# microsoft/DCVC

Measured on AMD Instinct MI355X. Metric: 1080p YUV420 intra encode+decode pictures per second (DCVC-UF-Intra (DMCI), real rANS bit streams, q_index in {0,16,32,48,63}; sequential loop: compress then decompress per picture), higher is better.
Workload: dtype f16

## Files before the change

dcvc_amd/csrc/codec/codec_base.h:

```cpp
#pragma once

#include "codec/modules.h"
#include "rans/rans_coder.h"

#include <initializer_list>
#include <condition_variable>
#include <functional>
#include <map>
#include <mutex>
#include <thread>

namespace dcvc {

constexpr int kMinSymbolsPerStream = 32768;
constexpr int kQpNum = 64;

inline int ceil_div(int a, int b) { return (a + b - 1) / b; }
inline int ec_parallel_for(int symbols)
{
    const int p = symbols / kMinSymbolsPerStream;
    return p < 1 ? 1 : (p > kMaxEcParallel ? kMaxEcParallel : p);
}

struct Geometry {
    int H8 = 0, W8 = 0, H16 = 0, W16 = 0, H16p = 0, W16p = 0, H32 = 0, W32 = 0, H64 = 0, W64 = 0;
    int P8() const { return H8 * W8; }
    int P16() const { return H16 * W16; }
    int P16p() const { return H16p * W16p; }
    int P32() const { return H32 * W32; }
    int P64() const { return H64 * W64; }
    bool padded() const { return H16p != H16 || W16p != W16; }

    static Geometry of(int height, int width)
    {
        Geometry g;
        g.H8 = ceil_div(height, 16) * 2; g.W8 = ceil_div(width, 16) * 2;
        g.H16 = g.H8 / 2; g.W16 = g.W8 / 2;
        g.H16p = ceil_div(g.H16, 4) * 4; g.W16p = ceil_div(g.W16, 4) * 4;
        g.H32 = g.H16p / 2; g.W32 = g.W16p / 2;
        g.H64 = g.H16p / 4; g.W64 = g.W16p / 4;
        return g;
    }
};

template <typename T>
class Pinned {
public:
    Pinned() = default;
    ~Pinned() { release(); }
    Pinned(const Pinned&) = delete;
    Pinned& operator=(const Pinned&) = delete;
    void reserve(size_t count)
    {
        if (count <= m_cap) return;
        release();
        hip_check(hipHostMalloc(reinterpret_cast<void**>(&m_p), count * sizeof(T), hipHostMallocDefault),
                  "hipHostMalloc");
        m_cap = count;
    }
    T* get() const { return m_p; }
    T& operator[](size_t i) const { return m_p[i]; }

private:
    void release()
    {
        if (m_p) (void)hipHostFree(m_p);
        m_p = nullptr;
        m_cap = 0;
    }
    T* m_p = nullptr;
    size_t m_cap = 0;
};

class CodecBase {
public:
    void set_use_graphs(bool on) { m_use_graphs = on; }
    const std::vector<uint8_t>& stream_bytes() const { return m_enc.stream(); }

protected:
    CodecBase();
    ~CodecBase();
    CodecBase(const CodecBase&) = delete;
    CodecBase& operator=(const CodecBase&) = delete;

    hipStream_t enter(hipStream_t user);
    void leave(hipStream_t user);

    template <typename F>
    void run_stage(int key, hipStream_t st, F&& fn);
    void bind_stage_arg(int key, const void* arg);
    void clear_graphs();
    void quiesce();

    void submit(hipStream_t st, std::function<void()> job);
    void wait_job();

    void load_cdf_tables(const ParamStore& ps);
    const half_t* upload_qp_table(const ParamStore& ps, DeviceArena& mem, const char* name, int ch);
    struct QpRow {
        half_t* dst;
        const half_t* table;
        int ch;
    };
    static void copy_qp_rows(std::initializer_list<QpRow> rows, int qp, hipStream_t st);

    void upload_code_length_tables(const ParamStore& ps, DeviceArena& mem, int ch_z, int max_n);
    void probe_code_length(int n, const int16_t* comp, long long comp_stride, int count, const int32_t* totals, int n_totals,
                           const int8_t* z, int nz, int qp, int64_t* units, int64_t* kept, hipStream_t st);

    RansEncoder m_enc;
    RansDecoder m_dec;
    hipStream_t m_io_stream = nullptr;
    hipStream_t m_cs = nullptr;
    hipStream_t m_join = nullptr;
    bool m_use_graphs = true;

private:
    const uint32_t *m_cl_y = nullptr, *m_cl_z = nullptr;
    int m_cl_y_num = 0, m_cl_z_num = 0, m_cl_ch_z = 0, m_cl_max_n = 0;
    unsigned long long* m_cl_sums = nullptr;
    Pinned<unsigned long long> m_h_cl;

    void worker_loop();

    struct GraphSlot {
        hipGraphExec_t exec = nullptr;
        bool warmed = false;
        const void* arg = nullptr;
    };
    std::map<int, GraphSlot> m_graphs;
    hipEvent_t m_ev_job = nullptr, m_ev_in = nullptr, m_ev_out = nullptr;
    std::thread m_worker;
    std::mutex m_mu;
    std::condition_variable m_cv_work, m_cv_done;
    std::function<void()> m_job;
    bool m_pending = false, m_done = true, m_stop = false;
    std::string m_worker_error;
};

template <typename F>
void CodecBase::run_stage(int key, hipStream_t st, F&& fn)
{
    if (!m_use_graphs) {
        fn();
        return;
    }
    GraphSlot& slot = m_graphs[key];
    if (!slot.warmed) {
        fn();
        slot.warmed = true;
        return;
    }
    if (!slot.exec) {
        hipGraph_t graph = nullptr;
// ... 18 lines not shown
```

dcvc_amd/csrc/codec/codec_base.hip:

```cpp
#include "codec/codec_base.h"

#include "rans/code_length.h"

#include <chrono>
#include <cstdio>
#include <cstdlib>
#include <string>

namespace dcvc {

CodecBase::CodecBase()
{
    int lo = 0, hi = 0;
    hip_check(hipDeviceGetStreamPriorityRange(&lo, &hi), "hipDeviceGetStreamPriorityRange");
    int prio = 0, io_prio = hi;
    if (const char* e = getenv("DCVC_COMPUTE_PRIORITY")) {
        const std::string v(e);
        prio = v == "high" ? hi : v == "low" ? lo : 0;
        io_prio = v == "low" ? lo : hi;
    }
    hip_check(hipStreamCreateWithPriority(&m_io_stream, hipStreamNonBlocking, io_prio), "hipStreamCreate(io)");
    hip_check(hipStreamCreateWithPriority(&m_cs, hipStreamNonBlocking, prio), "hipStreamCreate(compute)");
    hip_check(hipEventCreateWithFlags(&m_ev_job, hipEventDisableTiming), "hipEventCreate");
    hip_check(hipEventCreateWithFlags(&m_ev_in, hipEventDisableTiming), "hipEventCreate");
    hip_check(hipEventCreateWithFlags(&m_ev_out, hipEventDisableTiming), "hipEventCreate");
    m_worker = std::thread(&CodecBase::worker_loop, this);
}

CodecBase::~CodecBase()
{
    {
        std::lock_guard<std::mutex> lk(m_mu);
        m_stop = true;
    }
    m_cv_work.notify_all();
    if (m_worker.joinable()) m_worker.join();
    clear_graphs();
    if (m_cs) (void)hipStreamSynchronize(m_cs);
    if (m_ev_job) (void)hipEventDestroy(m_ev_job);
    if (m_ev_in) (void)hipEventDestroy(m_ev_in);
    if (m_ev_out) (void)hipEventDestroy(m_ev_out);
    if (m_join) (void)hipStreamDestroy(m_join);
    if (m_cs) (void)hipStreamDestroy(m_cs);
    if (m_io_stream) (void)hipStreamDestroy(m_io_stream);
}

void CodecBase::clear_graphs()
{
    for (auto& kv : m_graphs) {
        if (kv.second.exec) (void)hipGraphExecDestroy(kv.second.exec);
    }
    m_graphs.clear();
}

void CodecBase::quiesce()
{
    {
        std::unique_lock<std::mutex> lk(m_mu);
        m_cv_done.wait(lk, [&] { return m_done && !m_pending; });
    }
    if (m_cs) (void)hipStreamSynchronize(m_cs);
    if (m_io_stream) (void)hipStreamSynchronize(m_io_stream);
}

void CodecBase::bind_stage_arg(int key, const void* arg)
{
    GraphSlot& slot = m_graphs[key];
    if (slot.exec && slot.arg != arg) {
        (void)hipGraphExecDestroy(slot.exec);
        slot.exec = nullptr;
    }
    slot.arg = arg;
}

namespace {
bool join_by_blocking_stream()
{
    static const bool on = [] {
        const char* e = getenv("DCVC_NULL_STREAM_JOIN");
        return e == nullptr || std::string(e) != "event";
    }();
    return on;
}
}

hipStream_t CodecBase::enter(hipStream_t user)
{
    hip_check(hipEventRecord(m_ev_in, user), "hipEventRecord(in)");
    hip_check(hipStreamWaitEvent(m_cs, m_ev_in, 0), "hipStreamWaitEvent(in)");
    return m_cs;
}

// ... 169 lines not shown
```

dcvc_amd/csrc/codec/dmci.h:

```cpp
#pragma once

#include "codec/codec_base.h"

namespace dcvc {

class DmciCodec : public CodecBase {
public:
    static constexpr int kChSrc = 192, kChEncDec = 384, kChY = 256, kChZ = 128;

    DmciCodec();
    ~DmciCodec();

    void set_param(const ParamStore& ps, float skip_thres);

    int compress(const half_t* x, int height, int width, int qp, half_t* x_hat, hipStream_t stream);

    void decompress(const uint8_t* bits, size_t nbytes, int qp, int height, int width, int ec_parallel,
                    half_t* x_hat, hipStream_t stream);

    static constexpr int kMaxBatch = 16;
    void compress_batch(int n, const half_t* x, int height, int width, int qp, half_t* x_hat, int* ec_parallel_out,
                        hipStream_t stream);
    void decompress_batch(int n, const uint8_t* const* bits, const size_t* nbytes, const int* ec_parallel, int qp,
                          int height, int width, half_t* x_hat, hipStream_t stream);
    void estimate_bits(int n, const half_t* x, int height, int width, int qp, int64_t* units, int64_t* kept,
                       hipStream_t stream);
    int last_batch() const { return m_last_n; }
    const std::vector<uint8_t>& stream_at(int i) const;

    size_t debug_read(const std::string& name, void* dst, size_t cap, hipStream_t stream);

private:
    struct BatchGeometry : Geometry {
        int N = 0;
        int H = 0, W = 0;
    };

    void prepare(int height, int width, int n);
    void compress_impl(int n, const half_t* x, int height, int width, int qp, half_t* x_hat, hipStream_t user);
    void decompress_impl(int n, const uint8_t* const* bits, const size_t* nbytes, const int* ec_parallel, int qp,
                         int height, int width, half_t* x_hat, hipStream_t user);
    void select_qp(int qp, hipStream_t st);
    void run_encoder(hipStream_t st);
    void run_hyper_and_priors_enc(hipStream_t st);
    void run_priors_from_zhat(hipStream_t st);
    void run_spatial_prior(int k, hipStream_t st);
    void run_decoder(half_t* x_hat, hipStream_t st);
    void enc_stage0(hipStream_t st);
    void entropy_encode(int qp);

    DeviceArena m_wmem;
    const half_t* m_q_enc = nullptr;
    const half_t* m_q_dec = nullptr;
    const half_t* m_q_y_enc = nullptr;
    const half_t* m_q_y_dec = nullptr;
    half_t* m_zeros = nullptr;
    DcbW m_enc1, m_enc2[6];
    ConvKW m_enc_down;
    DcbW m_henc0;
    Stride2W m_henc1, m_henc2;
    UpsampleW m_hdec0, m_hdec1;
    DcbW m_hdec2;
    DcbW m_fus[3];
    FinW m_fus3;
    Conv1x1W m_reduction;
    DcbW m_sp_adaptor[3], m_sp[3];
    FinW m_sp3;
    UpsampleW m_dec_up;
    DcbW m_dec1[12], m_dec2;
    float m_skip_thres = 0.f;
    bool m_has_params = false;

    BatchGeometry m_g;
    DeviceArena m_bmem;
    Scratch m_s;
    half_t *m_U = nullptr, *m_F = nullptr, *m_Y = nullptr, *m_Ypad = nullptr;
    half_t *m_Z1 = nullptr, *m_Z2a = nullptr, *m_Z2 = nullptr, *m_Z3a = nullptr, *m_Z3 = nullptr, *m_ZH = nullptr;
    int8_t* m_ZI8 = nullptr;
    half_t *m_H1a = nullptr, *m_H1 = nullptr, *m_H2a = nullptr, *m_H2 = nullptr, *m_HP = nullptr;
    half_t *m_PF = nullptr, *m_PARAMSp = nullptr, *m_PARAMS = nullptr, *m_CAT = nullptr, *m_AD = nullptr, *m_SP = nullptr;
    half_t *m_YHAT = nullptr, *m_D0 = nullptr, *m_D1 = nullptr, *m_R = nullptr;
    half_t *m_cur_q_enc = nullptr, *m_cur_q_dec = nullptr, *m_cur_q_y_enc = nullptr, *m_cur_q_y_dec = nullptr;
    int16_t *m_SYM = nullptr, *m_COMP = nullptr;
    uint8_t *m_COND = nullptr, *m_IDX = nullptr, *m_CIDX = nullptr;
    int8_t* m_DECODED = nullptr;
    size_t m_idx_region = 0;
    int32_t *m_CNT = nullptr, *m_TOTALS = nullptr;
    Pinned<int32_t> m_h_totals;
    Pinned<int16_t> m_h_sym;
    Pinned<int8_t> m_h_z;
    Pinned<uint8_t> m_h_idx;
    Pinned<int8_t> m_h_dec;
    int m_ec_parallel = 1;
    int m_last_n = 0;
    std::vector<std::vector<uint8_t>> m_streams;
    std::vector<int> m_ec_parallels;
    std::vector<RansDecoder::StreamState> m_dec_states;
};

}
```

dcvc_amd/csrc/codec/dmci.hip:

```cpp
#include "codec/dmci.h"

#include <chrono>
#include <cstdio>
#include <cstdlib>

#include <algorithm>
#include <cstring>

namespace dcvc {

namespace {

enum StageKey : int { kEnc0 = 0, kEnc1 = 1, kDec0 = 10, kDec1 = 11 };

}

DmciCodec::DmciCodec() = default;

DmciCodec::~DmciCodec()
{
    quiesce();
}

void DmciCodec::set_param(const ParamStore& ps, float skip_thres)
// ... 2 lines not shown
    clear_graphs();
    m_wmem.release();
    kernels_init();
    m_skip_thres = skip_thres;
    m_q_enc = upload_qp_table(ps, m_wmem, "q_scale_enc", kChEncDec);
    m_q_dec = upload_qp_table(ps, m_wmem, "q_scale_dec", kChEncDec);
    m_q_y_enc = upload_qp_table(ps, m_wmem, "q_scale_y_enc", kChY);
    m_q_y_dec = upload_qp_table(ps, m_wmem, "q_scale_y_dec", kChY);
    m_zeros = m_wmem.alloc_half(2048);
    m_cur_q_enc = m_wmem.alloc_half(kChEncDec);
    m_cur_q_dec = m_wmem.alloc_half(kChEncDec);
    m_cur_q_y_enc = m_wmem.alloc_half(kChY);
    m_cur_q_y_dec = m_wmem.alloc_half(kChY);

    m_enc1.load(ps, m_wmem, "enc.enc_1.");
    for (int i = 0; i < 6; ++i) m_enc2[i].load(ps, m_wmem, "enc.enc_2." + std::to_string(i) + ".");
    m_enc_down.load(ps, m_wmem, "enc.enc_2.6.");
    m_henc0.load(ps, m_wmem, "hyper_enc.conv.0.");
    m_henc1.load(ps, m_wmem, "hyper_enc.conv.1.");
    m_henc2.load(ps, m_wmem, "hyper_enc.conv.2.");
    m_hdec0.load(ps, m_wmem, "hyper_dec.conv.0.");
    m_hdec1.load(ps, m_wmem, "hyper_dec.conv.1.");
    m_hdec2.load(ps, m_wmem, "hyper_dec.conv.2.");
    for (int i = 0; i < 3; ++i) m_fus[i].load(ps, m_wmem, "y_prior_fusion.conv." + std::to_string(i) + ".");
    m_fus3.load(ps, m_wmem, "y_prior_fusion.conv.3.");
    m_reduction.load(ps, m_wmem, "y_spatial_prior_reduction.");
    for (int i = 0; i < 3; ++i) {
        m_sp_adaptor[i].load(ps, m_wmem, "y_spatial_prior_adaptor_" + std::to_string(i + 1) + ".");
        m_sp[i].load(ps, m_wmem, "y_spatial_prior.conv." + std::to_string(i) + ".");
    }
    m_sp3.load(ps, m_wmem, "y_spatial_prior.conv.3.");
    m_dec_up.load(ps, m_wmem, "dec.dec_1.0.");
    for (int i = 0; i < 12; ++i) m_dec1[i].load(ps, m_wmem, "dec.dec_1." + std::to_string(i + 1) + ".");
    m_dec2.load(ps, m_wmem, "dec.dec_2.");

    load_cdf_tables(ps);
    upload_code_length_tables(ps, m_wmem, kChZ, kMaxBatch);
    m_has_params = true;
}

void DmciCodec::prepare(int height, int width, int n)
{
    if (!m_has_params) throw std::runtime_error("DMCI: set_param() has not been called");
    if (n < 1 || n > kMaxBatch) throw std::invalid_argument("DMCI: batch size must be in [1, 16]");
    if (m_g.H == height && m_g.W == width && m_g.N == n) return;
    quiesce();
    clear_graphs();
    m_bmem.release();
    m_g = BatchGeometry();
    BatchGeometry g;
    static_cast<Geometry&>(g) = Geometry::of(height, width);
    g.N = n;
    g.H = height; g.W = width;
    auto H = [&](size_t count) { return m_bmem.alloc_half(count); };
    const size_t N = n;
    const size_t P8 = N * g.P8(), P16 = N * g.P16(), P16p = N * g.P16p(), P32 = N * g.P32(), P64 = N * g.P64();
    m_s.elems = std::max<size_t>(P8 * kChEncDec, P16p * 2 * kChY);
    m_s.batch = n;
    m_s.t1 = H(m_s.elems); m_s.t2 = H(m_s.elems); m_s.t3 = H(m_s.elems);
    m_U = H(P8 * kChSrc); m_F = H(P8 * kChEncDec);
    m_Y = H(P16 * kChY); m_Ypad = g.padded() ? H(P16p * kChY) : m_Y;
    m_Z1 = H(P16p * kChZ); m_Z2a = H(P32 * kChZ); m_Z2 = H(P32 * kChZ);
    m_Z3a = H(P64 * kChZ); m_Z3 = H(P64 * kChZ); m_ZH = H(P64 * kChZ);
    m_ZI8 = static_cast<int8_t*>(m_bmem.alloc(P64 * kChZ));
    m_H1a = H(P32 * kChZ); m_H1 = H(P32 * kChZ); m_H2a = H(P16p * kChZ); m_H2 = H(P16p * kChZ);
    m_HP = H(P16p * kChY);
    m_PF = H(P16p * 2 * kChY); m_PARAMSp = H(P16p * 2 * kChY);
    m_PARAMS = g.padded() ? H(P16 * 2 * kChY) : m_PARAMSp;
    m_CAT = H(P16 * 2 * kChY); m_AD = H(P16 * 2 * kChY); m_SP = H(P16 * 2 * kChY);
    m_YHAT = H(P16 * kChY);
    m_D0 = H(P8 * kChEncDec); m_D1 = H(P8 * kChEncDec); m_R = H(P8 * kChSrc);
    const size_t nq = static_cast<size_t>(g.P16()) * (kChY / 4);
    m_SYM = static_cast<int16_t*>(m_bmem.alloc(N * nq * 2));
    m_COMP = static_cast<int16_t*>(m_bmem.alloc(N * 4 * nq * 2));
    m_COND = static_cast<uint8_t*>(m_bmem.alloc(N * nq / 8 + 8));
    m_IDX = static_cast<uint8_t*>(m_bmem.alloc(N * nq));
    m_idx_region = (16 + nq + 15) / 16 * 16;
    m_CIDX = static_cast<uint8_t*>(m_bmem.alloc(N * 4 * m_idx_region));
    m_DECODED = static_cast<int8_t*>(m_bmem.alloc(N * 4 * nq));
    m_CNT = static_cast<int32_t*>(m_bmem.alloc(sizeof(int32_t) * N * symbol_blocks(static_cast<int>(nq))));
    m_TOTALS = static_cast<int32_t*>(m_bmem.alloc(sizeof(int32_t) * 4 * N));
    m_h_totals.reserve(16 * N);
    m_h_sym.reserve(N * 4 * nq);
    m_h_z.reserve(P64 * kChZ + 64);
    m_h_idx.reserve(N * 4 * m_idx_region);
    m_h_dec.reserve(N * 4 * nq);
    m_g = g;
}

void DmciCodec::select_qp(int qp, hipStream_t st)
{
    copy_qp_rows({{m_cur_q_enc, m_q_enc, kChEncDec}, {m_cur_q_dec, m_q_dec, kChEncDec},
                  {m_cur_q_y_enc, m_q_y_enc, kChY}, {m_cur_q_y_dec, m_q_y_dec, kChY}}, qp, st);
}

void DmciCodec::run_encoder(hipStream_t st)
{
    const BatchGeometry& g = m_g;
    const View f(m_F, kChEncDec, kChEncDec);
    ChainCall enc1, enc2;
    enc1.q_after_last = m_cur_q_enc;
    enc1.after = m_enc1.feeds(m_enc2[0]) ? &m_enc2[0] : nullptr;
    enc2.first_dc0_done = enc1.after != nullptr;
    run_dcb_chain(&m_enc1, 1, View(m_U, kChSrc, kChSrc), f, f, g.H8, g.W8, m_s, st, enc1);
    run_dcb_chain(m_enc2, 6, f, f, f, g.H8, g.W8, m_s, st, enc2);
    ConvKxKDesc d;
    d.x = m_F; d.ldx = kChEncDec; d.w = m_enc_down.w; d.bias = m_enc_down.b; d.zeros = m_zeros;
    d.y = m_Y; d.ldy = kChY; d.in_h = g.H8; d.in_w = g.W8; d.cin = kChEncDec; d.cout = kChY;
    d.ksize = 3; d.stride = 2; d.pad = 1; d.n = g.N;
    conv_kxk(d, st);
}

void DmciCodec::run_hyper_and_priors_enc(hipStream_t st)
{
    const BatchGeometry& g = m_g;
    if (g.padded()) {
        replicate_pad_b(m_Y, kChY, g.H16, g.W16, kChY, g.H16p - g.H16, g.W16p - g.W16, m_Ypad, kChY, g.N, st);
    }
    m_henc0.forward(View(m_Ypad, kChY, kChY), View(m_Z1, kChZ, kChZ), g.H16p, g.W16p, m_s, st);
    m_henc1.forward(View(m_Z1, kChZ, kChZ), View(m_Z2a, kChZ, kChZ), View(m_Z2, kChZ, kChZ), g.H16p, g.W16p,
                    m_zeros, m_s, st);
    m_henc2.forward(View(m_Z2, kChZ, kChZ), View(m_Z3a, kChZ, kChZ), View(m_Z3, kChZ, kChZ), g.H32, g.W32,
                    m_zeros, m_s, st);
    round_z(m_Z3, m_ZH, m_ZI8, g.N * g.P64() * kChZ, st);
    run_priors_from_zhat(st);
}

void DmciCodec::run_priors_from_zhat(hipStream_t st)
{
    const BatchGeometry& g = m_g;
    m_hdec0.forward(View(m_ZH, kChZ, kChZ), View(m_H1a, kChZ, kChZ), View(m_H1, kChZ, kChZ), g.H64, g.W64, m_s, st);
    m_hdec1.forward(View(m_H1, kChZ, kChZ), View(m_H2a, kChZ, kChZ), View(m_H2, kChZ, kChZ), g.H32, g.W32, m_s, st);
    m_hdec2.forward(View(m_H2, kChZ, kChZ), View(m_HP, kChY, kChY), g.H16p, g.W16p, m_s, st);
    const View pf(m_PF, 2 * kChY, 2 * kChY);
    {
        const FinCall fin(m_fus3, m_PARAMSp, 2 * kChY);
        ChainCall fus;
        fus.fin = &fin;
        run_dcb_chain(m_fus, 3, View(m_HP, kChY, kChY), pf, pf, g.H16p, g.W16p, m_s, st, fus);
    }
    if (g.padded()) {
        crop_b(m_PARAMSp, 2 * kChY, g.H16p, g.W16p, m_PARAMS, 2 * kChY, g.H16, g.W16, 2 * kChY, g.N, st);
    }
    {
        Conv1x1Desc d;
        d.x = m_PARAMS; d.ldx = 2 * kChY; d.w = m_reduction.w; d.bias = m_reduction.b;
        d.y = m_CAT + kChY; d.ldy = 2 * kChY; d.pixels = g.N * g.P16(); d.cin = 2 * kChY; d.cout = kChY;
        conv1x1(d, st);
    }
}

void DmciCodec::run_spatial_prior(int k, hipStream_t st)
{
    const BatchGeometry& g = m_g;
    const View ad(m_AD, 2 * kChY, 2 * kChY);
    const FinCall fin(m_sp3, m_SP, 2 * kChY);
    ChainCall adaptor, sp;
    adaptor.after = m_sp_adaptor[k].feeds(m_sp[0]) ? &m_sp[0] : nullptr;
    sp.first_dc0_done = adaptor.after != nullptr;
    sp.fin = &fin;
    run_dcb_chain(&m_sp_adaptor[k], 1, View(m_CAT, 2 * kChY, 2 * kChY), ad, ad, g.H16, g.W16, m_s, st, adaptor);
    run_dcb_chain(m_sp, 3, ad, ad, ad, g.H16, g.W16, m_s, st, sp);
}

void DmciCodec::run_decoder(half_t* x_hat, hipStream_t st)
{
    const BatchGeometry& g = m_g;
    const View d1(m_D1, kChEncDec, kChEncDec);
    const DcbW* after_up = m_dec_up.block.feeds(m_dec1[0]) ? &m_dec1[0] : nullptr;
    m_dec_up.forward(View(m_YHAT, kChY, kChY), View(m_D0, kChEncDec, kChEncDec), d1, g.H16, g.W16, m_s, st, nullptr, nullptr,
                     after_up);
    ChainCall dec1;
    dec1.q_after_last = m_cur_q_dec;
    dec1.first_dc0_done = after_up != nullptr;
    run_dcb_chain(m_dec1, 12, d1, d1, d1, g.H8, g.W8, m_s, st, dec1);
    m_dec2.forward(d1, View(m_R, kChSrc, kChSrc), g.H8, g.W8, m_s, st);
    shuffle8_b(m_R, kChSrc, g.H8, g.W8, 3, true, x_hat, g.N, st);
}

void DmciCodec::enc_stage0(hipStream_t st)
{
    const BatchGeometry& g = m_g;
    run_encoder(st);
    run_hyper_and_priors_enc(st);
    mul_channel(m_Y, kChY, m_cur_q_y_enc, m_Y, kChY, g.N * g.P16(), kChY, st);
    const int nq = g.P16() * (kChY / 4);
    for (int k = 0; k < 4; ++k) {
        const half_t* prm = k == 0 ? m_PARAMS : m_SP;
        YStepEnc d;
        d.y = m_Y; d.ldy = kChY;
        d.scales = prm; d.lds = 2 * kChY;
        d.means = prm + kChY; d.ldm = 2 * kChY;
        d.y_hat_acc = m_CAT; d.ldacc = 2 * kChY;
        d.sym = m_SYM; d.cond = m_COND; d.block_count = m_CNT;
        d.H = g.H16; d.W = g.W16; d.C = kChY; d.step = k; d.skip_thres = m_skip_thres; d.first = (k == 0); d.n = g.N;
        y_step_enc(d, st);
        compact_b(m_SYM, 2, m_COND, m_CNT, nq, m_COMP, 4LL * nq, m_TOTALS, 4, k, g.N, st);
        if (k < 3) run_spatial_prior(k, st);
    }
    mul_channel(m_CAT, 2 * kChY, m_cur_q_y_dec, m_YHAT, kChY, g.N * g.P16(), kChY, st);
}

int DmciCodec::compress(const half_t* x, int height, int width, int qp, half_t* x_hat, hipStream_t user)
{
    compress_impl(1, x, height, width, qp, x_hat, user);
    return m_ec_parallel;
}

void DmciCodec::compress_batch(int n, const half_t* x, int height, int width, int qp, half_t* x_hat, int* ec_parallel_out,
                               hipStream_t user)
{
    compress_impl(n, x, height, width, qp, x_hat, user);
    for (int i = 0; i < n; ++i) ec_parallel_out[i] = i == 0 ? m_ec_parallel : m_ec_parallels[i];
}

const std::vector<uint8_t>& DmciCodec::stream_at(int i) const
{
    if (i < 0 || i >= m_last_n) throw std::invalid_argument("DMCI: no stream " + std::to_string(i) + " in the last call");
    return i == 0 ? stream_bytes() : m_streams[i];
}

void DmciCodec::compress_impl(int n, const half_t* x, int height, int width, int qp, half_t* x_hat, hipStream_t user)
{
    m_last_n = 0;
    prepare(height, width, n);
    hipStream_t st = enter(user);
    select_qp(qp, st);
    pad_unshuffle8_b(x, height, width, 3, m_U, m_g.H8, m_g.W8, n, st);
    run_stage(kEnc0, st, [&] { enc_stage0(st); });
    submit(st, [this, qp] { entropy_encode(qp); });
    bind_stage_arg(kEnc1, x_hat);
    run_stage(kEnc1, st, [&] { run_decoder(x_hat, st); });
    leave(user);
    wait_job();
    m_last_n = n;
}

void DmciCodec::estimate_bits(int n, const half_t* x, int height, int width, int qp, int64_t* units, int64_t* kept,
                              hipStream_t user)
{
    if (qp < 0 || qp >= kQpNum) throw std::invalid_argument("DMCI estimate_bits: qp must be in [0, 63]");
    prepare(height, width, n);
    const BatchGeometry& g = m_g;
    hipStream_t st = enter(user);
    select_qp(qp, st);
    pad_unshuffle8_b(x, height, width, 3, m_U, g.H8, g.W8, n, st);
    run_stage(kEnc0, st, [&] { enc_stage0(st); });
    const long long nq = static_cast<long long>(g.P16()) * (kChY / 4);
    probe_code_length(n, m_COMP, 4 * nq, static_cast<int>(4 * nq), m_TOTALS, 4, m_ZI8, g.P64() * kChZ, qp, units, kept, st);
    leave(user);
}

void DmciCodec::entropy_encode(int qp)
{
    const BatchGeometry& g = m_g;
    static const bool trace = getenv("DCVC_TIMING") != nullptr;
    const auto t_call = std::chrono::steady_clock::now();
    hip_check(hipMemcpyAsync(m_h_totals.get(), m_TOTALS, 4 * g.N * sizeof(int32_t), hipMemcpyDeviceToHost, m_io_stream), "D2H totals");
    const int nz = g.P64() * kChZ;
    const size_t nq = static_cast<size_t>(g.P16()) * (kChY / 4);
    hip_check(hipMemcpyAsync(m_h_z.get(), m_ZI8, static_cast<size_t>(g.N) * nz, hipMemcpyDeviceToHost, m_io_stream), "D2H z");
    hip_check(hipStreamSynchronize(m_io_stream), "sync io");
    bool copied = false;
    for (int b = 0; b < g.N; ++b) {
        int total = 0;
        for (int k = 0; k < 4; ++k) total += m_h_totals[4 * b + k];
        if (total > 0) {
            hip_check(hipMemcpyAsync(m_h_sym.get() + 4 * nq * b, m_COMP + 4 * nq * b, static_cast<size_t>(total) * 2,
                                     hipMemcpyDeviceToHost, m_io_stream), "D2H symbols");
            copied = true;
        }
    }
    if (copied) hip_check(hipStreamSynchronize(m_io_stream), "sync io");
    const auto t_coded = std::chrono::steady_clock::now();
    m_streams.resize(g.N);
    m_ec_parallels.resize(g.N);
    for (int b = g.N - 1; b >= 0; --b) {
        const int32_t* totals = m_h_totals.get() + 4 * b;
        const int16_t* sym = m_h_sym.get() + 4 * nq * b;
        int base[4], total = 0;
        for (int k = 0; k < 4; ++k) {
            base[k] = total;
            total += totals[k];
        }
        m_ec_parallel = ec_parallel_for(total);
        m_enc.reset();
        m_enc.set_parallel(m_ec_parallel);
        for (int k = 3; k >= 0; --k) m_enc.push_y(sym + base[k], totals[k]);
        m_enc.push_z(m_h_z.get() + static_cast<size_t>(nz) * b, nz, qp * kChZ, kChZ);
        m_enc.flush();
        m_ec_parallels[b] = m_ec_parallel;
        if (b > 0) m_streams[b] = m_enc.stream();
    }
    if (trace) {
        using us = std::chrono::duration<double, std::micro>;
        fprintf(stderr, "[dcvc] compress host entropy coding of %d pictures %.0f us (waiting for the GPU %.0f us)\n", g.N,
                us(std::chrono::steady_clock::now() - t_coded).count(), us(t_coded - t_call).count());
    }
}

void DmciCodec::decompress(const uint8_t* bits, size_t nbytes, int qp, int height, int width,
                           int ec_parallel, half_t* x_hat, hipStream_t user)
{
    decompress_impl(1, &bits, &nbytes, &ec_parallel, qp, height, width, x_hat, user);
}

void DmciCodec::decompress_batch(int n, const uint8_t* const* bits, const size_t* nbytes, const int* ec_parallel, int qp,
                                 int height, int width, half_t* x_hat, hipStream_t user)
{
    decompress_impl(n, bits, nbytes, ec_parallel, qp, height, width, x_hat, user);
}

void DmciCodec::decompress_impl(int n, const uint8_t* const* bits, const size_t* nbytes, const int* ec_parallel, int qp,
                                int height, int width, half_t* x_hat, hipStream_t user)
{
    prepare(height, width, n);
    const BatchGeometry& g = m_g;
    hipStream_t st = enter(user);
    select_qp(qp, st);
    const int nz = g.P64() * kChZ;
    const int nq = g.P16() * (kChY / 4);
    static const bool trace = getenv("DCVC_TIMING") != nullptr;
    using clk = std::chrono::steady_clock;
    auto us_since = [](clk::time_point t) { return std::chrono::duration<double, std::micro>(clk::now() - t).count(); };
    const auto t_call = clk::now();
    double us_rans = 0, us_wait = 0;
    long n_sym = 0;
    const bool turns = n > 1;
    if (turns) m_dec_states.resize(n);
    auto t_z = clk::now();
    for (int b = 0; b < n; ++b) {
        m_dec.set_parallel(ec_parallel[b]);
        m_dec.set_stream(bits[b], nbytes[b]);
        m_dec.decode_z(nz, qp * kChZ, kChZ, m_h_z.get() + static_cast<size_t>(nz) * b);
        if (turns) m_dec.swap_state(m_dec_states[b]);
    }
    us_rans += us_since(t_z);
    hip_check(hipMemcpyAsync(m_ZI8, m_h_z.get(), static_cast<size_t>(nz) * n, hipMemcpyHostToDevice, st), "H2D z");

    auto region_of = [&](int b, int k) { return static_cast<size_t>(b * 4 + k) * m_idx_region; };
    auto index_step = [&](int k) {
        YStepDecIndex d;
        d.scales = k == 0 ? m_PARAMS : m_SP; d.lds = 2 * kChY;
        d.index = m_IDX; d.cond = m_COND; d.block_count = m_CNT;
        d.H = g.H16; d.W = g.W16; d.C = kChY; d.step = k; d.skip_thres = m_skip_thres; d.n = n;
        y_step_dec_index(d, st);
        uint8_t* region = m_CIDX + region_of(0, k);
        compact_b(m_IDX, 1, m_COND, m_CNT, nq, region + 16, 4LL * static_cast<long long>(m_idx_region),
                  reinterpret_cast<int32_t*>(region), static_cast<int>(m_idx_region), 0, n, st);
    };
    run_stage(kDec0, st, [&] {
        int8_to_half(m_ZI8, m_ZH, n * nz, st);
        run_priors_from_zhat(st);
        index_step(0);
    });
    bind_stage_arg(kDec1 + 3, x_hat);
    static const size_t kFirst = [] { const char* e = getenv("DCVC_IDX_FIRST_KB"); return static_cast<size_t>(e ? atoi(e) : 192) * 1024; }();
    const size_t first = std::min(m_idx_region, 16 + kFirst);
    for (int k = 0; k < 4; ++k) {
        auto t_w = clk::now();
        for (int b = 0; b < n; ++b) {
            hip_check(hipMemcpyAsync(m_h_idx.get() + region_of(b, k), m_CIDX + region_of(b, k), first, hipMemcpyDeviceToHost, st),
                      "D2H count + indexes");
        }
        hip_check(hipStreamSynchronize(st), "sync");
        bool more = false;
        for (int b = 0; b < n; ++b) {
            uint8_t* h_region = m_h_idx.get() + region_of(b, k);
            const int cnt = *reinterpret_cast<const int32_t*>(h_region);
            if (cnt < 0 || cnt > nq) throw std::runtime_error("DMCI decompress: bad symbol count");
            if (16 + static_cast<size_t>(cnt) > first) {
                hip_check(hipMemcpyAsync(h_region + first, m_CIDX + region_of(b, k) + first, 16 + cnt - first,
                                         hipMemcpyDeviceToHost, st), "D2H indexes");
                more = true;
            }
        }
        if (more) hip_check(hipStreamSynchronize(st), "sync");
        us_wait += us_since(t_w);
        for (int b = 0; b < n; ++b) {
            const uint8_t* h_region = m_h_idx.get() + region_of(b, k);
            const int cnt = *reinterpret_cast<const int32_t*>(h_region);
            if (cnt == 0) continue;
            const size_t at = static_cast<size_t>(b * 4 + k) * nq;
            auto t_r = clk::now();
            if (turns) m_dec.swap_state(m_dec_states[b]);
            m_dec.decode_y(h_region + 16, cnt, m_h_dec.get() + at);
            if (turns) m_dec.swap_state(m_dec_states[b]);
            us_rans += us_since(t_r);
            n_sym += cnt;
            hip_check(hipMemcpyAsync(m_DECODED + at, m_h_dec.get() + at, cnt, hipMemcpyHostToDevice, st), "H2D symbols");
        }
        run_stage(kDec1 + k, st, [&] {
            YStepDecRestore d;
            d.decoded = m_DECODED + static_cast<size_t>(k) * nq; d.cond = m_COND; d.block_count = m_CNT;
            d.totals = reinterpret_cast<const int32_t*>(m_CIDX + region_of(0, k));
            d.slot = 0;
            d.n = n; d.decoded_stride = 4LL * nq; d.totals_stride = static_cast<int>(m_idx_region);
            d.means = (k == 0 ? m_PARAMS : m_SP) + kChY; d.ldm = 2 * kChY;
            d.y_hat_acc = m_CAT; d.ldacc = 2 * kChY;
            d.H = g.H16; d.W = g.W16; d.C = kChY; d.step = k; d.first = (k == 0);
            y_step_dec_restore(d, st);
            if (k < 3) {
                run_spatial_prior(k, st);
                index_step(k + 1);
            } else {
                mul_channel(m_CAT, 2 * kChY, m_cur_q_y_dec, m_YHAT, kChY, n * g.P16(), kChY, st);
                run_decoder(x_hat, st);
            }
        });
    }
    if (trace) {
        size_t bytes = 0;
        for (int b = 0; b < n; ++b) bytes += nbytes[b];
        fprintf(stderr, "[dcvc] decompress host %.0f us: entropy decoding %.0f us (%ld y symbols, %zu bytes, %d streams, "
                        "%d pictures), waiting for the GPU %.0f us\n", us_since(t_call), us_rans, n_sym, bytes, ec_parallel[0],
                n, us_wait);
    }
    leave(user);
}

size_t DmciCodec::debug_read(const std::string& name, void* dst, size_t cap, hipStream_t st)
{
    const BatchGeometry& g = m_g;
    const void* src = nullptr;
    size_t bytes = 0;
    if (name == "y") { src = m_Y; bytes = static_cast<size_t>(g.N) * g.P16() * kChY * 2; }
    else if (name == "y_hat") { src = m_YHAT; bytes = static_cast<size_t>(g.N) * g.P16() * kChY * 2; }
    else if (name == "z_i8") { src = m_ZI8; bytes = static_cast<size_t>(g.N) * g.P64() * kChZ; }
    else if (name == "params") { src = m_PARAMS; bytes = static_cast<size_t>(g.N) * g.P16() * 2 * kChY * 2; }
    else if (name == "unshuffled") { src = m_U; bytes = static_cast<size_t>(g.N) * g.P8() * kChSrc * 2; }
    else if (name == "features") { src = m_F; bytes = static_cast<size_t>(g.N) * g.P8() * kChEncDec * 2; }
    else if (name == "totals") { src = m_TOTALS; bytes = 16 * static_cast<size_t>(g.N); }
    else if (name == "symbols") { src = m_COMP; bytes = static_cast<size_t>(g.N) * g.P16() * kChY * 2; }
    else throw std::invalid_argument("unknown debug tensor '" + name + "'");
    if (dst != nullptr) {
        hip_check(hipStreamSynchronize(st), "sync");
        hip_check(hipStreamSynchronize(m_cs), "sync");
        hip_check(hipMemcpy(dst, src, std::min(bytes, cap), hipMemcpyDeviceToHost), "debug D2H");
    }
    return bytes;
}

}
```

dcvc_amd/csrc/rans/rans_coder.cpp:

```cpp
#include "rans_coder.h"

#include <chrono>
#if defined(__x86_64__)
#include <immintrin.h>
#endif
#include <cstdlib>

#include <algorithm>
#include <cassert>
#include <cstdio>
#include <cstring>
#include <numeric>
#include <stdexcept>

namespace dcvc {

namespace {

constexpr uint32_t kProbMask = (1u << kRansProbBits) - 1;
constexpr int kEncRenormShift = 23 - kRansProbBits + 8;
constexpr uint32_t kBypassMax = (1u << kBypassBits) - 1;
constexpr uint32_t kBypassFreqLimit = (1u << (kRansProbBits - kBypassBits)) << kEncRenormShift;

struct EncState {
// ... 217 lines not shown
void CdfTable::load(const int32_t* cdfs, int num_cdf, int row_stride, const int32_t* cdf_sizes)
{
    num = num_cdf;
    stride = row_stride;
    const size_t total = static_cast<size_t>(num) * stride;
    start.assign(total, 0);
    freq.assign(total, 0);
    rcp.assign(total, 0);
    rcp_shift.assign(total, 0);
    cdf.assign(total + 1, 0);
    max_value.assign(num, 0);
    for (int i = 0; i < num; ++i) {
        max_value[i] = static_cast<int8_t>(cdf_sizes[i] - 2);
        const int32_t* row = cdfs + static_cast<size_t>(i) * stride;
        for (int j = 0; j < stride; ++j) {
            cdf[static_cast<size_t>(i) * stride + j] = static_cast<uint32_t>(row[j]);
        }
        for (int j = 0; j + 1 < stride; ++j) {
            const size_t e = static_cast<size_t>(i) * stride + j;
            const uint32_t f = static_cast<uint16_t>(row[j + 1] - row[j]);
            start[e] = static_cast<uint16_t>(row[j]);
            freq[e] = static_cast<uint16_t>(f);
            if (f >= 2) {
                uint32_t shift = 0;
                while (f > (1u << shift)) {
                    ++shift;
                }
                rcp[e] = static_cast<uint32_t>(((1ull << (shift + 31)) + f - 1) / f);
                rcp_shift[e] = static_cast<uint8_t>(shift - 1);
            }
        }
    }
    edge.clear();
    bool vector_ok = stride <= kEdgeRow + 1 && kRansProbBits == 16 && cpu_has_avx512bw();
    for (int i = 0; vector_ok && i < num; ++i) {
        const uint32_t* row = cdf.data() + static_cast<size_t>(i) * stride;
        const int size = cdf_sizes[i];
        if (size < 2 || size > stride || row[0] != 0) vector_ok = false;
        for (int j = 1; vector_ok && j < size; ++j) {
            if (row[j] == 0 || row[j] < row[j - 1] || row[j] > (1u << kRansProbBits)) vector_ok = false;
        }
        if (vector_ok && row[size - 1] != (1u << kRansProbBits)) vector_ok = false;
    }
    if (!vector_ok && stride <= kEdgeRow + 1 && kRansProbBits == 16 && cpu_has_avx512bw() && getenv("DCVC_RANS_AVX512") == nullptr) {
        static bool said = false;
        if (!said) {
            said = true;
            fprintf(stderr, "[dcvc] rANS decoder: a CDF table (%d rows) is not of the form the vector search needs "
                            "(0 = cdf[0] < cdf[1] <= ... <= cdf[size - 1] = 65536): portable search for it\n", num);
        }
    }
    if (vector_ok) {
        edge.assign(static_cast<size_t>(num) * kEdgeRow, 0xFFFFu);
        for (int i = 0; i < num; ++i) {
            const uint32_t* row = cdf.data() + static_cast<size_t>(i) * stride;
            const int size = cdf_sizes[i];
            for (int j = 1; j < size && j <= kEdgeRow; ++j) {
                edge[static_cast<size_t>(i) * kEdgeRow + (j - 1)] = static_cast<uint16_t>(row[j] - 1u);
            }
        }
    }
    first.clear();
    if (num <= kLutRows && kRansProbBits == 16) {
        first.assign(static_cast<size_t>(num) * 256, 0);
        for (int i = 0; i < num; ++i) {
            const uint32_t* row = cdf.data() + static_cast<size_t>(i) * stride;
            const int last = cdf_sizes[i] - 2;
            int v = 0;
            for (uint32_t b = 0; b < 256; ++b) {
                while (v < last && row[v + 1] <= (b << 8)) ++v;
                first[static_cast<size_t>(i) * 256 + b] = static_cast<uint8_t>(v);
            }
        }
    }
}

namespace {
inline void cpu_relax()
{
#if defined(__x86_64__) || defined(__i386__)
    __builtin_ia32_pause();
#endif
}
}

WorkerPool::WorkerPool(int threads)
{
    if (const char* e = getenv("DCVC_RANS_SPIN_US")) m_spin_us = atoi(e);
    if (const char* e = getenv("DCVC_RANS_SPIN_WORKERS")) m_spin_workers = atoi(e);
    for (int i = 0; i < threads; ++i) {
        m_threads.emplace_back(&WorkerPool::loop, this, i);
    }
}

WorkerPool::~WorkerPool()
{
    {
        std::lock_guard<std::mutex> lk(m_mu);
        m_stop = true;
    }
    m_cv_work.notify_all();
    for (auto& t : m_threads) {
        t.join();
    }
}

void WorkerPool::loop(int index)
{
    const int spin_us = index < m_spin_workers ? m_spin_us : std::min(m_spin_us, 100);
    uint64_t seen = 0;
    std::unique_lock<std::mutex> lk(m_mu);
    for (;;) {
        m_cv_work.wait(lk, [&] { return m_stop || (m_epoch != seen && m_next < m_n); });
        if (m_stop) {
            return;
        }
        while (m_next < m_n) {
            const int item = m_next++;
            const auto* fn = m_fn;
            lk.unlock();
            std::exception_ptr err;
            try {
                (*fn)(item);
            } catch (...) {
                err = std::current_exception();
            }
            lk.lock();
            if (err && !m_error) {
                m_error = err;
            }
            m_pending_hint.store(--m_pending, std::memory_order_release);
            if (m_pending == 0) {
                m_cv_done.notify_all();
            }
        }
        seen = m_epoch;
        if (spin_us > 0 && !m_stop) {
            lk.unlock();
            const auto until = std::chrono::steady_clock::now() + std::chrono::microseconds(spin_us);
            while (m_epoch_hint.load(std::memory_order_acquire) == seen) {
                for (int i = 0; i < 64; ++i) cpu_relax();
                if (std::chrono::steady_clock::now() >= until) break;
            }
            lk.lock();
        }
    }
}

void WorkerPool::run(int n, const std::function<void(int)>& fn)
{
    if (n <= 0) {
        return;
    }
    if (n == 1 || m_threads.empty()) {
        for (int i = 0; i < n; ++i) {
            fn(i);
        }
        return;
    }
    std::unique_lock<std::mutex> lk(m_mu);
    m_fn = &fn;
    m_n = n;
    m_next = 1;
    m_pending = n;
    m_error = nullptr;
    ++m_epoch;
    m_pending_hint.store(n, std::memory_order_release);
    m_epoch_hint.store(m_epoch, std::memory_order_release);
    lk.unlock();
    m_cv_work.notify_all();
    auto guarded = [&](int item) {
        try {
            fn(item);
        } catch (...) {
            std::lock_guard<std::mutex> g(m_err_mu);
            if (!m_local_error) m_local_error = std::current_exception();
        }
    };
    m_local_error = nullptr;
    guarded(0);
    lk.lock();
    m_pending_hint.store(--m_pending, std::memory_order_release);
    while (m_next < m_n) {
        const int item = m_next++;
        lk.unlock();
        guarded(item);
        lk.lock();
        m_pending_hint.store(--m_pending, std::memory_order_release);
    }
    if (m_pending != 0 && m_spin_us > 0) {
        lk.unlock();
        const auto until = std::chrono::steady_clock::now() + std::chrono::microseconds(m_spin_us);
        while (m_pending_hint.load(std::memory_order_acquire) > 0) {
            for (int i = 0; i < 64; ++i) cpu_relax();
            if (std::chrono::steady_clock::now() >= until) break;
        }
        lk.lock();
    }
    m_cv_done.wait(lk, [&] { return m_pending == 0; });
    m_fn = nullptr;
    m_n = 0;
    std::exception_ptr err = m_local_error ? m_local_error : m_error;
    m_error = nullptr;
    m_local_error = nullptr;
    lk.unlock();
    if (err) {
        std::rethrow_exception(err);
    }
}

RansEncoder::RansEncoder() : m_pool(kMaxEcParallel - 1)
{
    m_buf.resize(kMaxEcParallel);
    m_begin.assign(kMaxEcParallel, 0);
}

void RansEncoder::set_cdf(const int32_t* cdfs, int num_cdf, int stride, const int32_t* cdf_sizes,
                          int index)
{
    if (index < 0 || index > 1) {
        throw std::invalid_argument("rANS table index must be 0 (z) or 1 (y)");
    }
    m_tab[index].load(cdfs, num_cdf, stride, cdf_sizes);
}

void RansEncoder::set_parallel(int n)
{
    if (n < 1 || n > kMaxEcParallel) {
        throw std::invalid_argument("entropy coder parallelism must be in [1, 8]");
    }
    m_n = n;
}

void RansEncoder::reset()
{
    m_segs.clear();
    m_out.clear();
}

void RansEncoder::push_y(const int16_t* symbols, int count)
{
    Segment s;
    s.y = symbols;
    s.count = count;
    m_segs.push_back(s);
}

void RansEncoder::push_z(const int8_t* symbols, int count, int cdf_offset, int ch)
{
    Segment s;
    s.z = symbols;
    s.count = count;
    s.cdf_offset = cdf_offset;
    s.ch = ch;
    m_segs.push_back(s);
}

void RansEncoder::encode_substream(int i)
{
    size_t symbols = 0;
    for (const Segment& seg : m_segs) {
        int b, len;
        slice_of(seg.count, m_n, i, b, len);
        symbols += static_cast<size_t>(len);
    }
    const size_t cap = symbols * 4 + 16;
    std::vector<uint8_t>& buf = m_buf[i];
    if (buf.size() < cap) {
        buf.resize(cap);
    }
    EncState st;
    st.r = kRansLow;
    st.p = buf.data() + buf.size();
    for (const Segment& seg : m_segs) {
        int b, len;
        slice_of(seg.count, m_n, i, b, len);
        if (seg.y != nullptr) {
            const CdfTable& t = m_tab[1];
            for (int k = b + len - 1; k >= b; --k) {
                const int16_t c = seg.y[k];
                enc_symbol(st, static_cast<int8_t>(c >> 8), t, c & 0xff);
            }
        } else {
            const CdfTable& t = m_tab[0];
// ... 237 lines not shown
```

dcvc_amd/csrc/rans/rans_coder.h:

```cpp
#pragma once

#include <atomic>
#include <condition_variable>
#include <cstddef>
#include <cstdint>
#include <exception>
#include <functional>
#include <mutex>
#include <cstdlib>
#include <new>
#include <thread>
#include <vector>

namespace dcvc {

constexpr int kMaxEcParallel = 8;
constexpr int kRansProbBits = 16;
constexpr uint32_t kRansLow = 1u << 23;
constexpr int kBypassBits = 2;

struct CdfTable {
    int num = 0;
    int stride = 0;
    std::vector<uint16_t> start;
    std::vector<uint16_t> freq;
    std::vector<uint32_t> rcp;
    std::vector<uint8_t> rcp_shift;
    std::vector<uint32_t> cdf;
    std::vector<int8_t> max_value;
    static constexpr int kLutRows = 256;
    std::vector<uint8_t> first;
    static constexpr int kEdgeRow = 32;
    template <class T> struct Aligned64 {
        using value_type = T;
        Aligned64() = default;
        template <class U> Aligned64(const Aligned64<U>&) {}
        T* allocate(size_t n) {
            void* p = std::aligned_alloc(64, (n * sizeof(T) + 63) / 64 * 64);
            if (!p) throw std::bad_alloc();
            return static_cast<T*>(p);
        }
        void deallocate(T* p, size_t) { std::free(p); }
        template <class U> bool operator==(const Aligned64<U>&) const { return true; }
        template <class U> bool operator!=(const Aligned64<U>&) const { return false; }
    };
    std::vector<uint16_t, Aligned64<uint16_t>> edge;
    void load(const int32_t* cdfs, int num_cdf, int row_stride, const int32_t* cdf_sizes);
};

class WorkerPool {
public:
    explicit WorkerPool(int threads);
    ~WorkerPool();
    void run(int n, const std::function<void(int)>& fn);

private:
    void loop(int tid);
    std::vector<std::thread> m_threads;
    std::mutex m_mu;
    std::condition_variable m_cv_work, m_cv_done;
    const std::function<void(int)>* m_fn = nullptr;
    int m_n = 0, m_next = 0, m_pending = 0;
    uint64_t m_epoch = 0;
    bool m_stop = false;
    std::atomic<uint64_t> m_epoch_hint{0};
    std::atomic<int> m_pending_hint{0};
    int m_spin_us = 1000;
    int m_spin_workers = 4;
    std::exception_ptr m_error, m_local_error;
    std::mutex m_err_mu;
};

class RansEncoder {
public:
    RansEncoder();
    void set_cdf(const int32_t* cdfs, int num_cdf, int stride, const int32_t* cdf_sizes, int index);
    void set_parallel(int n);
    int parallel() const { return m_n; }
    void reset();
    void push_y(const int16_t* symbols, int count);
    void push_z(const int8_t* symbols, int count, int cdf_offset, int ch);
    void flush();
    const std::vector<uint8_t>& stream() const { return m_out; }

private:
    struct Segment {
        const int16_t* y = nullptr;
        const int8_t* z = nullptr;
        int count = 0, cdf_offset = 0, ch = 1;
    };
    void encode_substream(int i);
    CdfTable m_tab[2];
    std::vector<Segment> m_segs;
    std::vector<std::vector<uint8_t>> m_buf;
    std::vector<size_t> m_begin;
    std::vector<uint8_t> m_out;
    int m_n = 1;
    WorkerPool m_pool;
};

class RansDecoder {
public:
    RansDecoder();
    void set_cdf(const int32_t* cdfs, int num_cdf, int stride, const int32_t* cdf_sizes, int index);
    void set_parallel(int n);
    void set_stream(const uint8_t* data, size_t size);
    void decode_y(const uint8_t* indexes, int count, int8_t* out);
    void decode_z(int count, int cdf_offset, int ch, int8_t* out);

private:
    struct Sub {
        std::vector<uint8_t> bytes;
        const uint8_t* ptr = nullptr;
        const uint8_t* end = nullptr;
        uint32_t state = 0;
    };

public:
    struct StreamState {
        Sub sub[kMaxEcParallel];
        int n = 1;
    };
    void swap_state(StreamState& s);

private:
    CdfTable m_tab[2];
    Sub m_sub[kMaxEcParallel];
    int m_n = 1;
    WorkerPool m_pool;
};

std::vector<uint32_t> pmf_to_quantized_cdf(const float* pmf, int n);

}
```

Baseline: 154.2.

## Use mapped coherent host memory for decode handoff instead of async copies

Decode buffers for z symbols, compacted indexes and decoded y symbols are allocated as mapped, coherent pinned host memory, and kernels read and write them directly through device pointers. This removes the per-step H2D and D2H memcpy calls between the GPU index/restore stages and the host rANS decoder. The cost is that kernels now reach host memory over the interconnect, with uncached coherent accesses. An env var keeps the old copy path, and timing instrumentation is added for worker-pool start lag and per-step waits.

```diff
diff --git a/dcvc_amd/csrc/codec/codec_base.h b/dcvc_amd/csrc/codec/codec_base.h
--- a/dcvc_amd/csrc/codec/codec_base.h
+++ b/dcvc_amd/csrc/codec/codec_base.h
@@ -3,6 +3,7 @@
 #include "codec/modules.h"
 #include "rans/rans_coder.h"
 
+#include <algorithm>
 #include <initializer_list>
 #include <condition_variable>
 #include <functional>
@@ -50,26 +51,38 @@
     ~Pinned() { release(); }
     Pinned(const Pinned&) = delete;
     Pinned& operator=(const Pinned&) = delete;
-    void reserve(size_t count)
-    {
-        if (count <= m_cap) return;
-        release();
-        hip_check(hipHostMalloc(reinterpret_cast<void**>(&m_p), count * sizeof(T), hipHostMallocDefault),
-                  "hipHostMalloc");
-        m_cap = count;
-    }
+    void reserve(size_t count) { grow(count, false); }
+    void reserve_mapped(size_t count) { grow(count, true); }
     T* get() const { return m_p; }
+    T* dev() const { return m_dev; }
     T& operator[](size_t i) const { return m_p[i]; }
 
 private:
+    void grow(size_t count, bool mapped)
+    {
+        if (count <= m_cap && (!mapped || m_dev != nullptr)) return;
+        count = std::max(count, m_cap);
+        release();
+        hip_check(hipHostMalloc(reinterpret_cast<void**>(&m_p), count * sizeof(T),
+                                mapped ? hipHostMallocMapped | hipHostMallocCoherent : hipHostMallocDefault), "hipHostMalloc");
+        m_cap = count;
+        if (mapped) hip_check(hipHostGetDevicePointer(reinterpret_cast<void**>(&m_dev), m_p, 0), "hipHostGetDevicePointer");
+    }
     void release()
     {
         if (m_p) (void)hipHostFree(m_p);
         m_p = nullptr;
+        m_dev = nullptr;
         m_cap = 0;
     }
     T* m_p = nullptr;
+    T* m_dev = nullptr;
     size_t m_cap = 0;
+};
+
+struct DecHandoff {
+    bool mapped = true;
+    static DecHandoff from_env();
 };
 
 class CodecBase {
diff --git a/dcvc_amd/csrc/codec/codec_base.hip b/dcvc_amd/csrc/codec/codec_base.hip
--- a/dcvc_amd/csrc/codec/codec_base.hip
+++ b/dcvc_amd/csrc/codec/codec_base.hip
@@ -8,6 +8,24 @@
 #include <string>
 
 namespace dcvc {
+
+DecHandoff DecHandoff::from_env()
+{
+    DecHandoff h;
+    const char* e = getenv("DCVC_DEC_HANDOFF");
+    if (e == nullptr) return h;
+    const std::string list(e);
+    for (size_t at = 0; at <= list.size();) {
+        const size_t end = std::min(list.find(',', at), list.size());
+        const std::string item = list.substr(at, end - at);
+        if (item == "copy" || item == "legacy") h.mapped = false;
+        if (!item.empty() && item != "copy" && item != "graphhead" && item != "coldworkers" && item != "legacy") {
+            throw std::invalid_argument("DCVC_DEC_HANDOFF: '" + item + "' is none of copy, graphhead, coldworkers, legacy");
+        }
+        at = end + 1;
+    }
+    return h;
+}
 
 CodecBase::CodecBase()
 {
diff --git a/dcvc_amd/csrc/codec/dmci.h b/dcvc_amd/csrc/codec/dmci.h
--- a/dcvc_amd/csrc/codec/dmci.h
+++ b/dcvc_amd/csrc/codec/dmci.h
@@ -91,6 +91,7 @@
     Pinned<int8_t> m_h_z;
     Pinned<uint8_t> m_h_idx;
     Pinned<int8_t> m_h_dec;
+    const DecHandoff m_handoff = DecHandoff::from_env();
     int m_ec_parallel = 1;
     int m_last_n = 0;
     std::vector<std::vector<uint8_t>> m_streams;
diff --git a/dcvc_amd/csrc/codec/dmci.hip b/dcvc_amd/csrc/codec/dmci.hip
--- a/dcvc_amd/csrc/codec/dmci.hip
+++ b/dcvc_amd/csrc/codec/dmci.hip
@@ -108,9 +108,15 @@
     m_TOTALS = static_cast<int32_t*>(m_bmem.alloc(sizeof(int32_t) * 4 * N));
     m_h_totals.reserve(16 * N);
     m_h_sym.reserve(N * 4 * nq);
-    m_h_z.reserve(P64 * kChZ + 64);
-    m_h_idx.reserve(N * 4 * m_idx_region);
-    m_h_dec.reserve(N * 4 * nq);
+    if (m_handoff.mapped) {
+        m_h_z.reserve_mapped(P64 * kChZ + 64);
+        m_h_idx.reserve_mapped(N * 4 * m_idx_region);
+        m_h_dec.reserve_mapped(N * 4 * nq);
+    } else {
+        m_h_z.reserve(P64 * kChZ + 64);
+        m_h_idx.reserve(N * 4 * m_idx_region);
+        m_h_dec.reserve(N * 4 * nq);
+    }
     m_g = g;
 }
 
@@ -259,6 +265,13 @@
     run_stage(kEnc1, st, [&] { run_decoder(x_hat, st); });
     leave(user);
     wait_job();
+    static const bool trace = getenv("DCVC_TIMING") != nullptr;
+    if (trace) {
+        const auto t0 = std::chrono::steady_clock::now();
+        hip_check(hipStreamSynchronize(st), "sync");
+        fprintf(stderr, "[dcvc] compress: reconstruction done %.0f us after the bit stream\n",
+                std::chrono::duration<double, std::micro>(std::chrono::steady_clock::now() - t0).count());
+    }
     m_last_n = n;
 }
 
@@ -351,7 +364,9 @@
     auto us_since = [](clk::time_point t) { return std::chrono::duration<double, std::micro>(clk::now() - t).count(); };
     const auto t_call = clk::now();
     double us_rans = 0, us_wait = 0;
+    double us_step[4][4] = {}, us_z_lag = 0;
     long n_sym = 0;
+    const bool mapped = m_handoff.mapped;
     const bool turns = n > 1;
     if (turns) m_dec_states.resize(n);
     auto t_z = clk::now();
@@ -359,11 +374,14 @@
         m_dec.set_parallel(ec_parallel[b]);
         m_dec.set_stream(bits[b], nbytes[b]);
         m_dec.decode_z(nz, qp * kChZ, kChZ, m_h_z.get() + static_cast<size_t>(nz) * b);
+        us_z_lag = std::max(us_z_lag, m_dec.pool().last_start_lag_us());
         if (turns) m_dec.swap_state(m_dec_states[b]);
     }
     us_rans += us_since(t_z);
-    hip_check(hipMemcpyAsync(m_ZI8, m_h_z.get(), static_cast<size_t>(nz) * n, hipMemcpyHostToDevice, st), "H2D z");
-
+    if (!mapped) hip_check(hipMemcpyAsync(m_ZI8, m_h_z.get(), static_cast<size_t>(nz) * n, hipMemcpyHostToDevice, st), "H2D z");
+
+    uint8_t* const d_idx = mapped ? m_h_idx.dev() : m_CIDX;
+    const int8_t* const d_dec = mapped ? m_h_dec.dev() : m_DECODED;
     auto region_of = [&](int b, int k) { return static_cast<size_t>(b * 4 + k) * m_idx_region; };
     auto index_step = [&](int k) {
         YStepDecIndex d;
@@ -371,12 +389,12 @@
         d.index = m_IDX; d.cond = m_COND; d.block_count = m_CNT;
         d.H = g.H16; d.W = g.W16; d.C = kChY; d.step = k; d.skip_thres = m_skip_thres; d.n = n;
         y_step_dec_index(d, st);
-        uint8_t* region = m_CIDX + region_of(0, k);
+        uint8_t* region = d_idx + region_of(0, k);
         compact_b(m_IDX, 1, m_COND, m_CNT, nq, region + 16, 4LL * static_cast<long long>(m_idx_region),
                   reinterpret_cast<int32_t*>(region), static_cast<int>(m_idx_region), 0, n, st);
     };
     run_stage(kDec0, st, [&] {
-        int8_to_half(m_ZI8, m_ZH, n * nz, st);
+        int8_to_half(mapped ? m_h_z.dev() : m_ZI8, m_ZH, n * nz, st);
         run_priors_from_zhat(st);
         index_step(0);
     });
@@ -385,7 +403,7 @@
     const size_t first = std::min(m_idx_region, 16 + kFirst);
     for (int k = 0; k < 4; ++k) {
         auto t_w = clk::now();
-        for (int b = 0; b < n; ++b) {
+        for (int b = 0; b < n && !mapped; ++b) {
             hip_check(hipMemcpyAsync(m_h_idx.get() + region_of(b, k), m_CIDX + region_of(b, k), first, hipMemcpyDeviceToHost, st),
                       "D2H count + indexes");
         }
@@ -395,14 +413,16 @@
             uint8_t* h_region = m_h_idx.get() + region_of(b, k);
             const int cnt = *reinterpret_cast<const int32_t*>(h_region);
             if (cnt < 0 || cnt > nq) throw std::runtime_error("DMCI decompress: bad symbol count");
-            if (16 + static_cast<size_t>(cnt) > first) {
+            if (!mapped && 16 + static_cast<size_t>(cnt) > first) {
                 hip_check(hipMemcpyAsync(h_region + first, m_CIDX + region_of(b, k) + first, 16 + cnt - first,
                                          hipMemcpyDeviceToHost, st), "D2H indexes");
                 more = true;
             }
         }
         if (more) hip_check(hipStreamSynchronize(st), "sync");
-        us_wait += us_since(t_w);
+        us_step[k][0] = us_since(t_w);
+        us_wait += us_step[k][0];
+        auto t_d = clk::now();
         for (int b = 0; b < n; ++b) {
             const uint8_t* h_region = m_h_idx.get() + region_of(b, k);
             const int cnt = *reinterpret_cast<const int32_t*>(h_region);
@@ -411,15 +431,18 @@
             auto t_r = clk::now();
             if (turns) m_dec.swap_state(m_dec_states[b]);
             m_dec.decode_y(h_region + 16, cnt, m_h_dec.get() + at);
+            us_step[k][2] = std::max(us_step[k][2], m_dec.pool().last_start_lag_us());
             if (turns) m_dec.swap_state(m_dec_states[b]);
             us_rans += us_since(t_r);
             n_sym += cnt;
-            hip_check(hipMemcpyAsync(m_DECODED + at, m_h_dec.get() + at, cnt, hipMemcpyHostToDevice, st), "H2D symbols");
+            if (!mapped) hip_check(hipMemcpyAsync(m_DECODED + at, m_h_dec.get() + at, cnt, hipMemcpyHostToDevice, st), "H2D symbols");
         }
+        us_step[k][1] = us_since(t_d);
+        auto t_e = clk::now();
         run_stage(kDec1 + k, st, [&] {
             YStepDecRestore d;
-            d.decoded = m_DECODED + static_cast<size_t>(k) * nq; d.cond = m_COND; d.block_count = m_CNT;
-            d.totals = reinterpret_cast<const int32_t*>(m_CIDX + region_of(0, k));
+            d.decoded = d_dec + static_cast<size_t>(k) * nq; d.cond = m_COND; d.block_count = m_CNT;
+            d.totals = reinterpret_cast<const int32_t*>(d_idx + region_of(0, k));
             d.slot = 0;
             d.n = n; d.decoded_stride = 4LL * nq; d.totals_stride = static_cast<int>(m_idx_region);
             d.means = (k == 0 ? m_PARAMS : m_SP) + kChY; d.ldm = 2 * kChY;
@@ -434,6 +457,7 @@
                 run_decoder(x_hat, st);
             }
         });
+        us_step[k][3] = us_since(t_e);
     }
     if (trace) {
         size_t bytes = 0;
@@ -441,6 +465,9 @@
         fprintf(stderr, "[dcvc] decompress host %.0f us: entropy decoding %.0f us (%ld y symbols, %zu bytes, %d streams, "
                         "%d pictures), waiting for the GPU %.0f us\n", us_since(t_call), us_rans, n_sym, bytes, ec_parallel[0],
                 n, us_wait);
+        fprintf(stderr, "[dcvc] decompress steps (us: wait decode start-lag enqueue):");
+        for (int k = 0; k < 4; ++k) fprintf(stderr, " k%d %.0f %.0f %.0f %.0f |", k, us_step[k][0], us_step[k][1], us_step[k][2], us_step[k][3]);
+        fprintf(stderr, " z start-lag %.0f\n", us_z_lag);
     }
     leave(user);
 }
diff --git a/dcvc_amd/csrc/rans/rans_coder.cpp b/dcvc_amd/csrc/rans/rans_coder.cpp
--- a/dcvc_amd/csrc/rans/rans_coder.cpp
+++ b/dcvc_amd/csrc/rans/rans_coder.cpp
@@ -323,6 +323,18 @@
     __builtin_ia32_pause();
 #endif
 }
+inline int64_t steady_ns()
+{
+    return std::chrono::duration_cast<std::chrono::nanoseconds>(std::chrono::steady_clock::now().time_since_epoch()).count();
+}
+}
+
+void WorkerPool::note_start()
+{
+    const int64_t t = steady_ns();
+    int64_t seen = m_start_max.load(std::memory_order_relaxed);
+    while (t > seen && !m_start_max.compare_exchange_weak(seen, t, std::memory_order_relaxed)) {
+    }
 }
 
 WorkerPool::WorkerPool(int threads)
@@ -361,6 +373,7 @@
             const auto* fn = m_fn;
             lk.unlock();
             std::exception_ptr err;
+            note_start();
             try {
                 (*fn)(item);
             } catch (...) {
@@ -394,11 +407,14 @@
         return;
     }
     if (n == 1 || m_threads.empty()) {
+        m_start_lag_ns = 0;
         for (int i = 0; i < n; ++i) {
             fn(i);
         }
         return;
     }
+    const int64_t t_entry = steady_ns();
+    m_start_max.store(t_entry, std::memory_order_relaxed);
     std::unique_lock<std::mutex> lk(m_mu);
     m_fn = &fn;
     m_n = n;
@@ -411,6 +427,7 @@
     lk.unlock();
     m_cv_work.notify_all();
     auto guarded = [&](int item) {
+        if (item > 0) note_start();
         try {
             fn(item);
         } catch (...) {
@@ -441,6 +458,7 @@
     m_cv_done.wait(lk, [&] { return m_pending == 0; });
     m_fn = nullptr;
     m_n = 0;
+    m_start_lag_ns = m_start_max.load(std::memory_order_relaxed) - t_entry;
     std::exception_ptr err = m_local_error ? m_local_error : m_error;
     m_error = nullptr;
     m_local_error = nullptr;
diff --git a/dcvc_amd/csrc/rans/rans_coder.h b/dcvc_amd/csrc/rans/rans_coder.h
--- a/dcvc_amd/csrc/rans/rans_coder.h
+++ b/dcvc_amd/csrc/rans/rans_coder.h
@@ -53,9 +53,13 @@
     explicit WorkerPool(int threads);
     ~WorkerPool();
     void run(int n, const std::function<void(int)>& fn);
+    double last_start_lag_us() const { return 1e-3 * static_cast<double>(m_start_lag_ns); }
 
 private:
     void loop(int tid);
+    void note_start();
+    std::atomic<int64_t> m_start_max{0};
+    int64_t m_start_lag_ns = 0;
     std::vector<std::thread> m_threads;
     std::mutex m_mu;
     std::condition_variable m_cv_work, m_cv_done;
@@ -107,6 +111,7 @@
     void set_stream(const uint8_t* data, size_t size);
     void decode_y(const uint8_t* indexes, int count, int8_t* out);
     void decode_z(int count, int cdf_offset, int ch, int8_t* out);
+    const WorkerPool& pool() const { return m_pool; }
 
 private:
     struct Sub {
```

Measured after the change: 156.6, median of 6. 1.5% higher.
